# jhorstmann/queryengine

Hardware: AMD Instinct MI355X
Metric: rows/sec filter+project over int64/f64 batch; achieved HBM GB/s in roofline (higher is better)
Workload: dtype int64/f64

## Files before the change

### queryengine_amd/csrc/qe_api.cpp

```cpp
#include <algorithm>
#include <cmath>
#include <cstdio>
#include <cstdlib>
#include <functional>
#include <sstream>

#include "qe_exec.h"
#include "qe_kernels.h"
#include "qe_pernode.h"
#include "qe_scan.h"

using namespace qe;

namespace {

constexpr double kDenseFromSelectivity = 0.12;
constexpr double kLocalUpToSelectivity = 0.03;
constexpr int64_t kSampleFromRows = 8ll << 20;

FusedGeometry geometry_of(const qe_ctx *ctx) {
    FusedGeometry g;
    const int t = ctx->opts.tuning[0], u = ctx->opts.tuning[1];
    if (t == 64 || t == 128 || t == 256 || t == 512 || t == 1024) g.threads = t;
    const int mw = ctx->opts.tuning[3] / 100;
// ... 31 lines not shown
    void partitioned_tile_512_threads();
    void hashed_unroll();
    void dense_lds_tile();
    void ring_lds_budget();
    void register_estimate();
    void compile_without_scratch();
};


}

namespace qe {

std::shared_ptr<Plan> get_plan(qe_ctx *ctx, const qe_batch *batch, const PlanRequest &rq) {
    if (rq.nproj < 0 || (rq.nproj > 0 && !rq.projs)) fail(QE_ERR_INVALID_ARG, "bad projection list");
    CodegenInput in;
    in.filter = rq.filter ? &rq.filter->e : nullptr;
    for (int32_t i = 0; i < rq.nproj; i++) {
        if (!rq.projs[i]) fail(QE_ERR_INVALID_ARG, "null projection");
        in.projections.push_back(&rq.projs[i]->e);
        if (rq.agg_fns) {
            if (rq.agg_fns[i] < QE_AGG_MIN || rq.agg_fns[i] > QE_AGG_AVG) fail(QE_ERR_UNSUPPORTED, "unsupported aggregation function");
            in.agg_fns.push_back(rq.agg_fns[i]);
        }
    }
    for (int32_t i = 0; i < rq.nkeys; i++) {
        if (!rq.keys || !rq.keys[i]) fail(QE_ERR_INVALID_ARG, "null group key");
        in.group_keys.push_back(&rq.keys[i]->e);
    }
    in.cmp_semantics = ctx->opts.cmp_semantics;
    if (rq.conj_order) in.conj_order = *rq.conj_order;
    in.hp_parts = rq.hp_parts;
    static const int lines_maxp = std::getenv("QE_HP_LINES_MAXP") ? std::atoi(std::getenv("QE_HP_LINES_MAXP")) : 512;
    in.hp_lines = !debug_bit(ctx, kDbgHpRecords) && rq.hp_parts <= lines_maxp ? 1 : 0;
    in.hp_shift = rq.hp_shift;
    in.geo = geometry_of(ctx);
    const bool wide = rq.geo_cand == 1;
    if (wide) {
        in.geo.unroll = 16;
        in.geo.subs_per_chunk = 4;
        in.geo.ring_entries = 512;
    } else if (rq.geo_cand == 2) {
        in.geo.unroll = 8;
        in.geo.subs_per_chunk = 8;
        in.geo.ring_entries = 512;
        in.geo.threads = 128;
    }
    in.nontemporal = ctx->opts.tuning[2] % 10 == 2 ? 0 : 1;
    in.vec_stores = ctx->opts.tuning[2] % 10 == 5 ? 1 : 0;
    in.nt_stores = ctx->opts.tuning[2] % 10 == 3 ? 0 : ctx->opts.tuning[2] % 10 == 4 ? 2 : 1;
    in.debug_mask = ctx->opts.tuning[5] & kDbgAblationMask;
    in.staged = !debug_bit(ctx, kDbgNoLateMaterialisation);
    in.prefetch = debug_bit(ctx, kDbgNoPrefetch) ? 0 : debug_bit(ctx, kDbgAlwaysPrefetch) ? 2 : 1;
    in.dense = rq.dense && rq.filter != nullptr && !rq.agg_fns;
    if (in.dense) {
        in.geo.subs_per_chunk = 1;
        in.geo.stagger = 0;
        if (ctx->opts.tuning[0] == 0) in.geo.threads = 256;
        if (ctx->opts.tuning[1] == 0) in.geo.unroll = 8;
    }
    in.filter_load_stages = debug_bit(ctx, kDbgOneFilterLoadStage) ? 1 : 0;
    std::ostringstream key;
    key << "m" << (rq.agg_fns ? 1 : 0) << (in.dense ? "D" : "") << "c" << in.cmp_semantics << "t" << in.geo.threads << "u" << in.geo.unroll << "s"
        << in.geo.subs_per_chunk << "n" << in.nontemporal << in.nt_stores << in.vec_stores << "L" << (in.staged ? 1 : 0) << "P" << in.prefetch << "." << in.filter_load_stages << "k" << in.geo.lookback_k << "G" << in.geo.gate_period_log2 << "." << in.geo.gate_width_log2 << "d" << in.debug_mask << "r" << in.geo.resolve_at << "g" << in.geo.stagger << "w" << in.geo.min_waves << "p" << in.geo.prio_mode << "b" << in.geo.nbuf << "R" << in.geo.ring_entries << "|";
    for (const Column &c : batch->cols) {
        in.schema.push_back(BoundColumn{c.type, c.validity != nullptr, c.dict});
        key << c.type << (c.validity ? 'n' : 'v') << (c.dict ? c.dict->id : 0) << ",";
    }
    auto add_prog = [&](const Expr *e) {
        key << "|";
        if (e) key.write((const char *)e->program.data(), (std::streamsize)e->program.size());
    };
    add_prog(in.filter);
    for (const Expr *e : in.projections) add_prog(e);
    for (const Expr *e : in.group_keys) {
        key << "|k";
        add_prog(e);
    }
    if (rq.agg_fns)
        for (int a : in.agg_fns) key << "|a" << a;
    if (in.hp_parts) key << "|H" << in.hp_parts << "." << in.hp_shift << "." << in.hp_lines;
    if (!in.conj_order.empty()) {
        key << "|O";
        for (int o : in.conj_order) key << o << ".";
    }
    const std::string k = key.str();
    auto it = ctx->plans.find(k);
    if (it != ctx->plans.end() && (it->second->kernel.fn || !rq.load)) return it->second;
    auto plan = std::make_shared<Plan>();
    PlanGeometry pg{ctx, in, plan.get(), wide, rq.agg_fns};
    pg.analyze();
    pg.narrow_plan_wide_candidate();
    pg.lds_table_1024_threads();
    pg.hash_partitioned_tile();
    pg.partitioned_tile_512_threads();
    pg.hashed_unroll();
    pg.dense_lds_tile();
    pg.ring_lds_budget();
    if (ctx->opts.tuning[3] / 100 == 0) {
        pg.register_estimate();
        pg.compile_without_scratch();
    } else {
        plan->cg = generate_fused_source(in);
    }
    plan->geo = in.geo;
    plan->explicit_geometry = ctx->opts.tuning[0] != 0 || ctx->opts.tuning[1] != 0 || ctx->opts.tuning[3] != 0 || ctx->opts.tuning[4] != 0 ||
                              ctx->opts.tuning[7] != 0;
    plan->aggregate = rq.agg_fns != nullptr;
    plan->kernel = ctx->jit->get(plan->cg.source, "qe_fused", rq.load);
    ctx->plans[k] = plan;
    return plan;
}

}

namespace {

// ... 857 lines not shown
```

### queryengine_amd/csrc/qe_codegen.cpp

```cpp
#include "qe_expr_rules.h"

#include <algorithm>
#include <cinttypes>
#include <cmath>
#include <cstdio>
#include <sstream>

namespace qe {

namespace {

const char *kPrelude1 = R"QE(
// ---- generated by libqe_hip: fused filter+project kernel for gfx950 ----
typedef unsigned long long u64;
typedef long long i64;
typedef unsigned int u32;
typedef double  qe_f64x2 __attribute__((ext_vector_type(2)));
typedef i64     qe_i64x2 __attribute__((ext_vector_type(2)));
typedef int     qe_i32x2 __attribute__((ext_vector_type(2)));
typedef u64     u64x2 __attribute__((ext_vector_type(2)));
// Bitmap words (validity, BOOLEAN values) are wave-uniform: read through the constant address space they become SCALAR loads
// (s_load_dwordx4 into SGPRs).  As plain global loads hipcc issued one 16-byte VECTOR load per group and bitmap in which all 64
// lanes fetch the same two words into four VGPRs each -- 48 VGPRs per sub-tile for three nullable columns.  The batch is
// read-only while a kernel runs and the scalar cache starts every kernel invalidated.
// ... 581 lines not shown
            if (a.k.empty()) return a;
            if (n.type == QE_STRING) r.dict = unify(a, b);
            r.v = "(" + a.k + " ? " + a.v + " : " + b.v + ")";
            if (!b.k.empty()) r.k = "(" + a.k + " || " + b.k + ")";
            r.from_int = a.from_int && b.from_int;
            return bind(r);
        }
        case QE_FN_ABS: {
            Val a = emit(e, n.ops[0]);
            r.k = a.k;
            if (n.type == QE_DOUBLE) r.v = "__builtin_fabs(" + a.v + ")";
            else if (n.type == QE_INT64) r.v = "(" + a.v + " < 0 ? (i64)(0ull - (u64)" + a.v + ") : " + a.v + ")";
            else r.v = "(" + a.v + " < 0 ? (int)(0u - (u32)" + a.v + ") : " + a.v + ")";
            r.from_int = a.from_int;
            return bind(r);
        }
        case QE_FN_FLOOR: case QE_FN_CEIL: {
            Val a = emit(e, n.ops[0]);
            if (n.type != QE_DOUBLE) return a;
            r.k = a.k;
            r.v = std::string(n.fn == QE_FN_FLOOR ? "floor(" : "ceil(") + a.v + ")";
            r.from_int = a.from_int;
            return bind(r);
        }
        case QE_FN_IN: case QE_FN_LIKE: return emit_member(e, n, id);
        default: fail(QE_ERR_INTERNAL, "bad function");
        }
    }
};

std::string load_vec_type(int t) {
    switch (t) {
    case QE_DOUBLE: return "qe_f64x2";
    case QE_INT64: return "qe_i64x2";
    default: return "qe_i32x2";
    }
}

void literal_to_dictionary(Val &v) {
    if (!v.is_str_lit) return;
    v.dict = literal_dictionary(v.lit);
    v.v = "0";
    v.is_str_lit = false;
}

enum class FusedForm { FilterProject, Dense, Aggregate, GroupByTable, GroupByPartitioned, GroupByHashed };

struct FusedAnalysis {
    CodegenOutput out;
    FusedForm form = FusedForm::FilterProject;
    bool aggregate = false, groupby = false, has_filter = false;
    bool staged = false;
    bool prefetch = false;
    std::string row_body;
    std::vector<std::string> conj_body;
    std::vector<int> col_stage;
    std::vector<int> vbit;
    std::vector<char> vonly;
    bool any_nullable_in = false;
    bool keys_nullable = false;
    bool member_bits = false, member_hash = false;
    std::string hp_grp_fn;
    HpEntryLayout hp_layout;
    bool row_grp() const { return groupby && !out.hashed; }
    bool row_keys() const { return groupby && (out.hashed || out.hp); }
};

FusedAnalysis analyze_fused(const CodegenInput &in);

struct Emitter {
    const CodegenInput &in;
    const FusedAnalysis &a;
    const CodegenOutput &out;
    const int NC, NO;
    std::ostringstream s;

    Emitter(const CodegenInput &i, const FusedAnalysis &an)
        : in(i), a(an), out(an.out), NC((int)an.out.used_cols.size()), NO((int)an.out.outs.size()) {}
    const BoundColumn &col(int j) const { return in.schema[(size_t)out.used_cols[(size_t)j]]; }

    void header();
    void groupby_macros();
    void access_macros();
    void row_functions();
    std::string valid_arg(int j) const;
    void loads(int stage, bool guarded);
    std::string col_args() const;
    void row_call(bool only_alive);
    void sub_head(const char *intro, const std::string &params, bool filter_project, bool scatter_pass);

    void filter_project();
    void dense();
    void filter_project_head();
    void ring_defs();
    void prefetch_loader();
    void compaction_tail();
    void passthrough_tail();
    void conj_probe();
    void ring_kernel();
    void two_pass_and_local();
    void aggregate();
    void groupby_table();
    void groupby_partitioned();
    void groupby_hashed();
    void hashed_prelude();
    void scatter_save_tail();
    void hashed_build_tail();
    void hashed_accumulate_tail();
    void partitioned_prelude();
    void group_rows_begin();
    void table_accumulate();
    void table_kernel();
    void gb_init_function(const char *comment);
    void merge_entry(const std::string &e);
    void partition_passes();
    void hp_aggregate_pass();
    void range_aggregate_pass();
};

FusedAnalysis analyze_fused(const CodegenInput &in) {
    Gen g(in);
    FusedAnalysis a;
    CodegenOutput &out = a.out;
    if (in.filter) g.mark_used(*in.filter);
    for (const Expr *p : in.projections) g.mark_used(*p);
    for (const Expr *k : in.group_keys) g.mark_used(*k);
    if ((int)g.used_cols.size() > kMaxCols) fail(QE_ERR_UNSUPPORTED, "too many input columns");
    if ((int)in.projections.size() > kMaxOuts) fail(QE_ERR_UNSUPPORTED, "too many projections");
    const bool aggregate = a.aggregate = !in.agg_fns.empty();

    int out_nconj = 0;
    std::vector<std::vector<int>> conj_cols;
    std::vector<int> conj;
    std::vector<std::string> &conj_body = a.conj_body;
    std::vector<int> &col_stage = a.col_stage;
    const bool staged = a.staged = in.filter != nullptr && in.staged && !in.dense;
    std::string keep_expr = "true";
    if (in.filter) {
        if (in.filter->nodes[in.filter->root].type != QE_BOOLEAN)
// ... 145 lines not shown
        out.table_words = 1 + 2 * (int)in.projections.size();
        out.hash_words = 3 + (int)in.group_keys.size() + 2 * (int)in.projections.size();
        {
            int shared = -1;
            for (size_t i = 0; i < out.outs.size(); i++) {
                if (out.outs[i].nullable) { out.cnt_src.push_back((int)i); continue; }
                if (shared < 0) shared = (int)i;
                out.cnt_src.push_back(shared);
            }
        }
        out.table_in_lds = !out.hashed && !out.hp && (size_t)out.ngroups * out.table_words * 8 <= (size_t)(in.geo.threads >= 1024 ? 144 : 48) * 1024;
        out.table_copies = 1;
        if (!out.hashed && !out.table_in_lds && in.projections.size() <= 8) {
            int shift = 0;
            static const size_t table_kb = std::getenv("QE_GB_TABLE_KB") ? (size_t)std::atoi(std::getenv("QE_GB_TABLE_KB")) : 80;
            while (shift < 12 && ((size_t)2 << shift) * out.table_words * 8 <= table_kb * 1024) shift++;
            if (out.hp) shift = out.hp_shift;
            const long long np = (out.ngroups + (1ll << shift) - 1) >> shift;
            if (np <= 1024) {
                for (size_t i = 0; i < in.projections.size(); i++) {
                    int slot = -1;
                    for (size_t j = 0; j < i; j++)
                        if (in.projections[j]->program == in.projections[i]->program) { slot = out.val_slot[j]; break; }
                    if (slot < 0) slot = out.nvals++;
                    out.val_slot.push_back(slot);
                }
                if (out.hp) {
                    out.hp_key_slot = out.nvals;
                    out.nvals += out.hp_key_words;
                    out.hp_line_recs = in.hp_lines ? 128 / (8 * out.nvals + 5) : 0;
                    if (out.hp_line_recs < 2) {
                        out.hp_line_recs = 0;
                        while (((1 + out.nvals) & out.nvals) != 0) out.nvals++;
                    }
                    if (((size_t)1 << out.hp_shift) * (size_t)(out.hp_key_words + 1 + hp_layout.words) * 8 > 156 * 1024)
                        fail(QE_ERR_UNSUPPORTED, "hash-partitioned GROUP BY: entry too wide for an LDS table");
                }
                out.partitioned = true;
                out.part_shift = shift;
                out.part_groups = 1 << shift;
                out.nparts = (int)np;
            }
        }
    }
    const int NC = (int)g.used_cols.size();
    a.vbit.assign((size_t)NC, -1);
    {
        int nn = 0;
        for (int j = 0; j < NC; j++)
            if (in.schema[g.used_cols[j]].nullable) a.vbit[j] = 2 * nn++;
        if (nn > 16) fail(QE_ERR_UNSUPPORTED, "more than 16 nullable input columns in one plan");
        a.any_nullable_in = nn > 0;
    }
    if (!groupby && !aggregate && staged && in.prefetch) {
        bool first = false;
        std::vector<char> has((size_t)conj.size() + 1, 0);
        for (int j = 0; j < NC; j++) { has[(size_t)col_stage[j]] = 1; first = first || col_stage[j] == 0; }
        int nstages = 0;
        for (char h : has) nstages += h ? 1 : 0;
        a.prefetch = first && (in.prefetch >= 2 ? nstages >= 2 : nstages >= 4);
    }
    out.used_cols = g.used_cols;
    out.aux_tables = g.aux;
    if (g.used_cols.size() + g.aux.size() > (size_t)kMaxCols)
        fail(QE_ERR_UNSUPPORTED, "too many input columns + string lookup tables for one fused kernel (use QE_EXEC_PER_NODE)");
    a.has_filter = out.has_filter = in.filter != nullptr;
    out.nconj = out_nconj;
    out.conj_cols = conj_cols;
    for (int j = 0; j < NC; j++) {
        a.vonly.push_back(g.value_used[(size_t)g.used_cols[j]] ? 0 : 1);
        out.col_width.push_back(a.vonly[(size_t)j] ? 0 : value_bytes(in.schema[g.used_cols[j]].type));
    }
    a.row_body = g.body.str();
    a.member_bits = g.uses_member_bits;
    a.member_hash = g.uses_member_hash;
    if (!aggregate) {
        out.dense = in.dense && a.has_filter;
        out.two_pass = a.has_filter && !out.dense;
        out.has_probe = staged && conj.size() >= 2;
        out.fl_ring = std::max(in.geo.ring_entries, output_row_bytes(out.outs) <= 18 ? 512 : 256);
        a.form = out.dense ? FusedForm::Dense : FusedForm::FilterProject;
    } else if (!groupby) {
        a.form = FusedForm::Aggregate;
    } else {
        a.form = out.hashed ? FusedForm::GroupByHashed : out.partitioned ? FusedForm::GroupByPartitioned : FusedForm::GroupByTable;
    }
    return a;
}

void Emitter::header() {
    const FusedGeometry &geo = in.geo;
    const int U = geo.unroll;
    s << "#define QE_LB_K " << geo.lookback_k << "\n#define QE_DEBUG_MASK " << in.debug_mask << "\n#define QE_RESOLVE_AT "
      << geo.resolve_at << "u\n#define QE_MIN_WAVES " << geo.min_waves << "\n#define QE_PRIO_MODE " << geo.prio_mode
      << "\n#define QE_PRIO_MOD " << (geo.prio_mode == 3 ? 2 : 3) << "u\n";
    s << kPrelude1;
    if (a.member_bits) s << kMemberBitsHelper;
    if (a.member_hash) s << kMemberHashHelper;
    s << "#define QE_THREADS " << geo.threads << "\n#define QE_WAVES " << geo.threads / 64 << "\n#define QE_U " << U
      << "\n#define QE_SUB_ROWS " << geo.sub_rows() << "\n#define QE_CHUNK_ROWS " << geo.chunk_rows() << "\n#define QE_SLOT_ROWS "
      << geo.slot_rows() << "\n#define QE_SUBS_PER_CHUNK " << geo.subs_per_chunk << "u\n#define QE_GATE_PERIOD "
      << (geo.gate_period_log2 > 0 ? (1u << geo.gate_period_log2) : 0u) << "u\n#define QE_GATE_WIDTH "
      << (geo.gate_period_log2 > 0 ? (1u << geo.gate_width_log2) : 0u) << "u\n";
}

void Emitter::groupby_macros() {
    s << "#define QE_GB_ADD_U64(p, v) atomicAdd((p), (v))\n#define QE_GB_ADD_F64(p, v) atomicAdd((p), (v))\n"
         "#define QE_GB_MIN_U64(p, v) atomicMin((p), (v))\n#define QE_GB_MIN_I64(p, v) atomicMin((p), (v))\n"
         "#define QE_GB_MAX_I64(p, v) atomicMax((p), (v))\n";
    s << "#define QE_GB_COPIES " << out.table_copies << "\n";
}

void Emitter::hashed_prelude() {
// ... 463 lines not shown
#if QE_GB_LINES
                    {
                        const u32 line = slot / QE_GB_PADU, idx = slot - line * QE_GB_PADU;
                        u64 *ln = L.stage + (size_t)line * 16;
                        if (QE_GB_NV % 2 == 0) {
#pragma unroll
                            for (int v = 0; v < QE_GB_NV; v += 2) {
                                u64x2 rv;
                                rv.x = sv.val[v][u][r];
                                rv.y = sv.val[v + 1 < QE_GB_NV ? v + 1 : v][u][r];
                                *(u64x2 *)(ln + idx * QE_GB_NV + v) = rv;
                            }
                        } else {
#pragma unroll
                            for (int v = 0; v < QE_GB_NV; ++v) ln[idx * QE_GB_NV + v] = sv.val[v][u][r];
                        }
                        ((u32 *)(ln + QE_GB_META))[idx] = (u32)(tile0 + (i64)(wave * QE_SUB_ROWS + u * 128 + 2 * lane + r));
                        if (QE_GB_FLAGS) ((unsigned char *)(ln + QE_GB_META) + 4u * QE_GB_PADU)[idx] = (unsigned char)(w & 255u);
                        if (idx == 0u) L.lineglob[line] = pos / QE_GB_PADU;   // (a run fills its lines from slot 0 on)
                        continue;
                    }
#endif
                    const u64 h = ((u64)pos << 32) | ((u64)(u32)(wave * QE_SUB_ROWS + u * 128 + 2 * lane + r) << (8 + QE_GB_SHIFT)) | ((u64)((w >> 9) & (QE_GB_GP - 1u)) << 8) | (u64)(w & 255u);
                    if (QE_GB_RECW % 2 == 0) {
                        u64x2 rv;
                        rv.x = h;
                        rv.y = sv.val[0][u][r];
                        *(u64x2 *)(L.stage + (size_t)slot * QE_GB_RECW) = rv;
#pragma unroll
                        for (int w = 2; w < QE_GB_RECW; w += 2) {   // record word w (>= 1) is value w - 1
                            u64x2 r2;
                            r2.x = sv.val[w - 1][u][r];
                            r2.y = sv.val[w][u][r];
                            *(u64x2 *)(L.stage + (size_t)slot * QE_GB_RECW + w) = r2;
                        }
                    } else {
                        L.stage[(size_t)slot * QE_GB_RECW] = h;
#pragma unroll
                        for (int v = 0; v < QE_GB_NV; ++v) L.stage[(size_t)slot * QE_GB_RECW + 1 + v] = sv.val[v][u][r];
                    }
                }
            }
        }
    }
}
)QE";
}

void Emitter::access_macros() {
    s << (in.nontemporal ? "#define QE_LD(p) __builtin_nontemporal_load(p)\n" : "#define QE_LD(p) (*(p))\n");
    s << (in.nt_stores ? "#define QE_ST(p, v) __builtin_nontemporal_store((v), (p))\n" : "#define QE_ST(p, v) (*(p) = (v))\n");
    s << (in.nt_stores == 2 ? "#define QE_SPILL_ST(p, v) __builtin_nontemporal_store((v), (p))\n" : "#define QE_SPILL_ST(p, v) (*(p) = (v))\n");
    s << "#define QE_VEC_ST " << (in.vec_stores ? 1 : 0) << "\n";
}

void Emitter::row_functions() {
    for (size_t ci = 0; ci < a.conj_body.size(); ci++) {
        s << "\n__device__ __forceinline__ void qe_conj" << ci << "(const QeParams &p, ";
        for (int j = 0; j < NC; j++) {
            const BoundColumn &bc = col(j);
            s << "const " << ctype(bc.type) << " c" << j << ", ";
            if (bc.nullable) s << "const bool kc" << j << ", ";
        }
        s << "bool &alive) {\n    (void)p;\n";
        for (int j = 0; j < NC; j++) {
            s << "    (void)c" << j << ";";
            if (col(j).nullable) s << " (void)kc" << j << ";";
        }
        s << "\n" << a.conj_body[ci] << "}\n";
    }
    s << "\n__device__ __forceinline__ void qe_row(const QeParams &p";
    bool first = false;
    for (int j = 0; j < NC; j++) {
        const BoundColumn &bc = col(j);
        s << (first ? "" : ", ") << "const " << ctype(bc.type) << " c" << j;
        first = false;
        if (bc.nullable) s << ", const bool kc" << j;
    }
    s << (first ? "" : ", ") << "bool &keep";
    for (int i = 0; i < NO; i++) {
        s << ", " << ctype(out.outs[i].type) << " &o" << i;
        if (out.outs[i].nullable) s << ", bool &ok" << i;
    }
    if (a.row_grp()) s << ", int &grp";
    if (a.row_keys()) {
        for (size_t i = 0; i < in.group_keys.size(); i++) s << ", u64 &kw" << i;
        s << ", u32 &knull";
    }
    s << ") {\n    (void)p;\n" << a.row_body << "}\n";
}

void Emitter::ring_defs() {
    const FusedGeometry &geo = in.geo;
    s << "\n#define QE_NBUF " << geo.nbuf << "u\n#define QE_RING " << geo.ring_entries << "   // LDS entries per wave, buffer and output column (power of two)\n";
    s << "#define QE_FL_RING " << out.fl_ring << "\n";
    s << "struct QeRing {\n";
    for (int i = 0; i < NO; i++) {
        const OutSpec &os = out.outs[i];
        s << "    " << (os.type == QE_BOOLEAN ? "unsigned char" : ctype(os.type)) << " *r" << i << ";\n";
        if (os.nullable) s << "    unsigned char *rv" << i << ";\n";
    }
    if (NO == 0) s << "    int unused;\n";
    s << "};\n";
}

std::string Emitter::valid_arg(int j) const { return "((qe_vb[u] >> (" + std::to_string(a.vbit[j]) + " + r)) & 1u) != 0u"; }

void Emitter::loads(int stage, bool guarded) {
    s << "#pragma unroll\n    for (int u = 0; u < QE_U; ++u) {\n";
    s << "        const i64 r0 = sub0 + u * 128 + 2 * lane;\n";
    s << "        const i64 g0 = (sub0 + u * 128) >> 6;   // wave-uniform bitmap word index (even)\n";
    s << "        const u32 sh = (u32)(2 * lane) & 63u;\n";
    s << "        const i64 nwords = (p.nrows + 63) >> 6;\n        (void)nwords; (void)g0; (void)sh; (void)r0;\n";
    if (guarded) s << "        if (keep[u][0] || keep[u][1]) {\n";
    for (int j = 0; j < NC; j++) {
        if (stage >= 0 && a.col_stage[j] != stage) continue;
        const BoundColumn &bc = col(j);
        auto bitmap_load = [&](const std::string &ptr, const std::string &dst, int vb = -1) {
            s << "        {\n            const qe_cu64p bm = (qe_cu64p)(u64)(" << ptr << ");\n";
            s << "            u64 w0, w1;\n";
            s << "            if (FULL) { w0 = bm[g0]; w1 = bm[g0 + 1]; }\n";
            s << "            else { w0 = g0 < nwords ? bm[g0] : 0ull; w1 = g0 + 1 < nwords ? bm[g0 + 1] : 0ull; }\n";
            s << "            const u64 w = lane < 32 ? w0 : w1;\n";
            if (vb >= 0) {
                s << "            qe_vb[u] |= ((u32)(w >> sh) & 3u) << " << vb << ";\n        }\n";
            } else {
                s << "            " << dst << "[u][0] = (w >> sh) & 1ull;\n";
                s << "            " << dst << "[u][1] = (w >> (sh + 1u)) & 1ull;\n        }\n";
            }
        };
        if (a.vonly[(size_t)j]) {
            const std::string ct = bc.type == QE_BOOLEAN ? "bool" : ctype(bc.type);
            s << "        c" << j << "[u][0] = (" << ct << ")0; c" << j << "[u][1] = (" << ct << ")0;\n";
        } else if (bc.type == QE_BOOLEAN) {
            bitmap_load("(const u64 *)p.col[" + std::to_string(j) + "]", "c" + std::to_string(j));
        } else {
            const std::string ct = ctype(bc.type), vt = load_vec_type(bc.type);
            s << "        {\n            const " << ct << " *src = (const " << ct << " *)p.col[" << j << "] + r0;\n";
            s << "            if (FULL) { const " << vt << " v = QE_LD((const " << vt << " *)src); c" << j
              << "[u][0] = v.x; c" << j << "[u][1] = v.y; }\n";
            s << "            else { c" << j << "[u][0] = r0 < p.nrows ? src[0] : (" << ct << ")0; c" << j
              << "[u][1] = r0 + 1 < p.nrows ? src[1] : (" << ct << ")0; }\n        }\n";
        }
        if (bc.nullable) bitmap_load("p.colvalid[" + std::to_string(j) + "]", "", a.vbit[j]);
    }
    if (guarded) s << "        }\n";
    s << "    }\n";
}

void Emitter::prefetch_loader() {
    bool s0_nulls = false;
    s << "\nstruct QeS0 {\n";
    for (int j = 0; j < NC; j++) {
        if (a.col_stage[j] != 0) continue;
        const BoundColumn &bc = col(j);
        s << "    " << (bc.type == QE_BOOLEAN ? "bool" : ctype(bc.type)) << " c" << j << "[QE_U][2];\n";
        s0_nulls = s0_nulls || bc.nullable;
    }
    if (s0_nulls) s << "    u32 vb[QE_U];\n";
    s << "};\n// issue the stage-0 loads of the (full) sub-tile at sub0\n"
         "__device__ __forceinline__ void qe_s0_load(const QeParams &p, const i64 sub0, const int lane, QeS0 &s0) {\n"
         "    constexpr bool FULL = true;\n";
    for (int j = 0; j < NC; j++)
        if (a.col_stage[j] == 0) s << "    auto &c" << j << " = s0.c" << j << ";\n";
    if (s0_nulls) s << "    auto &qe_vb = s0.vb;\n#pragma unroll\n    for (int u = 0; u < QE_U; ++u) qe_vb[u] = 0u;\n";
    loads(0, false);
    s << "}\n";
}

std::string Emitter::col_args() const {
    std::string args;
    for (int j = 0; j < NC; j++) {
        args += (args.empty() ? "" : ", ") + std::string("c") + std::to_string(j) + "[u][r]";
        if (col(j).nullable) args += ", " + valid_arg(j);
    }
    return args;
}

void Emitter::row_call(bool only_alive) {
    s << "#pragma unroll\n    for (int u = 0; u < QE_U; ++u) {\n#pragma unroll\n        for (int r = 0; r < 2; ++r) {\n";
    const std::string ca = col_args();
    if (only_alive) s << "            if (keep[u][r]) {\n                bool unused_keep;\n                qe_row(p, " << ca << (ca.empty() ? "" : ", ") << "unused_keep";
    else s << "            qe_row(p, " << ca << (ca.empty() ? "" : ", ") << "keep[u][r]";
    for (int i = 0; i < NO; i++) {
        s << ", o" << i << "[u][r]";
        if (out.outs[i].nullable) s << ", ok" << i << "[u][r]";
    }
    if (a.row_grp()) s << ", grp[u][r]";
    if (a.row_keys()) {
        for (size_t i = 0; i < in.group_keys.size(); i++) s << ", kw" << i << "[u][r]";
        s << ", knull[u][r]";
    }
    s << ");\n";
    if (only_alive) s << "                (void)unused_keep;\n            }\n";
    else s << "            if (!FULL) keep[u][r] = keep[u][r] && (sub0 + u * 128 + 2 * lane + r < p.nrows);\n";
    s << "        }\n    }\n";
}

const char *kPlainSubIntro = "\ntemplate <bool FULL, typename Hook>\n__device__ __forceinline__ void qe_sub(const QeParams &p, const i64 sub0, const int lane, Hook &&after_loads";

void Emitter::sub_head(const char *intro, const std::string &params, bool filter_project, bool scatter_pass) {
    s << intro << params << ") {\n";
    s << "    bool keep[QE_U][2];\n";
    if (a.row_grp()) s << "    int grp[QE_U][2];\n";
    if (a.row_keys()) {
        for (size_t i = 0; i < in.group_keys.size(); i++) s << "    u64 kw" << i << "[QE_U][2];\n";
        s << "    u32 knull[QE_U][2];\n";
    }
    for (int i = 0; i < NO; i++) {
        s << "    " << ctype(out.outs[i].type) << " o" << i << "[QE_U][2];\n";
        if (out.outs[i].nullable) s << "    bool ok" << i << "[QE_U][2];\n";
    }
    for (int j = 0; j < NC; j++) {
        const BoundColumn &bc = col(j);
        if (bc.type == QE_BOOLEAN) s << "    bool c" << j << "[QE_U][2];\n";
        else s << "    " << ctype(bc.type) << " c" << j << "[QE_U][2];\n";
    }
    if (a.any_nullable_in) s << "    u32 qe_vb[QE_U] = {};\n";
    if (!a.staged) {
        if (filter_project) s << "    (void)pf; (void)next_sub0;\n";
        loads(-1, false);
        s << "    after_loads();   // stores and polls of earlier work are issued here, under the loads just started\n";
        row_call(false);
    } else {
        const int K = (int)a.conj_body.size();
        for (int st = 0; st <= K; st++) {
            bool any = false;
            for (int j = 0; j < NC; j++) any = any || a.col_stage[j] == st;
            if (st == 0) {
                if (a.prefetch) {
                    s << "    if (PF) {   // stage 0 is in `pf` already; start the next sub-tile's stage 0 right away\n";
                    bool s0_nulls = false;
                    for (int j = 0; j < NC; j++) {
                        if (a.col_stage[j] != 0) continue;
                        s << "#pragma unroll\n        for (int u = 0; u < QE_U; ++u) { c" << j << "[u][0] = pf.c" << j << "[u][0]; c" << j << "[u][1] = pf.c" << j << "[u][1]; }\n";
                        s0_nulls = s0_nulls || col(j).nullable;
                    }
                    if (s0_nulls) s << "#pragma unroll\n        for (int u = 0; u < QE_U; ++u) qe_vb[u] = pf.vb[u];\n";
                    s << "        if (next_sub0 >= 0) qe_s0_load(p, next_sub0, lane, pf);\n    } else {\n";
                }
                loads(0, false);
                if (a.prefetch) s << "    }\n";
                if (!a.prefetch && filter_project) s << "    (void)pf; (void)next_sub0;\n";
                if (scatter_pass) {
                    s << "    if (MODE == 2) {\n";
                    for (int later = 1; later <= K; later++) {
                        bool has = false;
                        for (int j = 0; j < NC; j++) has = has || a.col_stage[j] == later;
                        if (has) loads(later, false);
                    }
                    s << "    }\n";
                }
                s << "    after_loads();   // stores and polls of earlier work are issued here, under the loads just started\n";
            } else if (any) {
                if (scatter_pass) s << "    if (MODE != 2) {\n";
                loads(st, true);
                if (scatter_pass) s << "    }\n";
            }
            if (st == K) break;
            s << "#pragma unroll\n    for (int u = 0; u < QE_U; ++u) {\n#pragma unroll\n        for (int r = 0; r < 2; ++r) {\n";
            const std::string ca = col_args();
            if (st == 0) {
                s << "            bool alive;\n            qe_conj0(p, " << ca << (ca.empty() ? "" : ", ") << "alive);\n";
                s << "            if (!FULL) alive = alive && (sub0 + u * 128 + 2 * lane + r < p.nrows);\n";
                s << "            keep[u][r] = alive;\n";
            } else {
                s << "            if (keep[u][r]) {\n                bool alive;\n                qe_conj" << st << "(p, " << ca << (ca.empty() ? "" : ", ")
                  << "alive);\n                keep[u][r] = alive;\n            }\n";
            }
            s << "        }\n    }\n";
        }
        row_call(true);
    }
}

void Emitter::scatter_save_tail() {
    s << "    if (MODE == 2) {   // keep the evaluated sub-tile: it is sorted and written under the next sub-tile's loads\n"
         "        sv.sub0 = sub0;\n#pragma unroll\n        for (int u = 0; u < QE_U; ++u) {\n#pragma unroll\n            for (int r = 0; r < 2; ++r) {\n"
         "                u32 w = ((u32)grp[u][r] << 9) | 256u;\n";
    for (int i = 0; i < NO; i++) {
        std::string cond = out.outs[i].nullable ? "ok" + std::to_string(i) + "[u][r]" : "true";
        s << "                if (" << cond << ") w |= " << (1u << i) << "u;\n";
    }
    s << "                sv.w[u][r] = keep[u][r] ? w : 0u;\n";
    {
        std::vector<std::string> slot_val((size_t)out.nvals);
        for (int i = NO - 1; i >= 0; i--) slot_val[out.val_slot[i]] = "__builtin_bit_cast(u64, (double)o" + std::to_string(i) + "[u][r])";
        if (out.hp) {
            for (int kk = 0; kk < (int)in.group_keys.size(); kk++) slot_val[(size_t)(out.hp_key_slot + kk)] = "kw" + std::to_string(kk) + "[u][r]";
            if (out.hp_key_words > (int)in.group_keys.size()) slot_val[(size_t)(out.hp_key_slot + out.hp_key_words - 1)] = "(u64)knull[u][r]";
        }
        for (int v = 0; v < out.nvals; v++) s << "                sv.val[" << v << "][u][r] = " << (slot_val[v].empty() ? std::string("0ull") : slot_val[v]) << ";\n";
    }
    s << "            }\n        }\n        return;\n    }\n";
}

void Emitter::hashed_build_tail() {
    s << "    if (MODE == 1) {\n        u32 id[QE_U][2];\n        u64 hh[QE_U][2], st[QE_U][2], ekn[QE_U][2], eid[QE_U][2], ek[QE_U][2][QE_HT_NK];\n        bool miss[QE_U][2];\n"
         "#pragma unroll\n        for (int u = 0; u < QE_U; ++u) {\n#pragma unroll\n            for (int r = 0; r < 2; ++r) {\n"
         "                miss[u][r] = keep[u][r]; id[u][r] = 0u; hh[u][r] = 0ull; st[u][r] = 0ull; ekn[u][r] = 0ull; eid[u][r] = 0ull;\n"
         "                if (keep[u][r]) {\n                    u64 key[QE_HT_NK];\n";
    for (size_t i = 0; i < in.group_keys.size(); i++) s << "                    key[" << i << "] = kw" << i << "[u][r];\n";
    s << "                    hh[u][r] = qe_ht_hash(key, (u64)knull[u][r]);\n"
         "                }\n            }\n        }\n"
         "        // up to 8 slots of the probe sequence, every pending row's loads in flight together per step\n"
         "        bool pend[QE_U][2], found[QE_U][2];\n        u32 slot[QE_U][2];\n"
         "#pragma unroll\n        for (int u = 0; u < QE_U; ++u) {\n#pragma unroll\n            for (int r = 0; r < 2; ++r) {\n"
         "                pend[u][r] = miss[u][r]; found[u][r] = false; slot[u][r] = (u32)hh[u][r] & ((u32)p.capacity - 1u) & ~3u;   // probe sequences start on a 4-entry group: one 128-byte line\n            }\n        }\n"
         "        if (QE_HT_NK == 1) {\n"
         "#pragma unroll\n            for (int u = 0; u < QE_U; ++u) {\n#pragma unroll\n                for (int r = 0; r < 2; ++r) slot[u][r] = (u32)hh[u][r] & ((u32)p.capacity - 1u) & ~7u;\n            }\n"
         "#pragma unroll\n            for (int d = 0; d < 8; ++d) {\n"
         "                bool anyp = false;\n"
         "#pragma unroll\n                for (int u = 0; u < QE_U; ++u) anyp = anyp || pend[u][0] || pend[u][1];\n"
         "                if (__ballot(anyp) == 0ull || (QE_DEBUG_MASK & 2)) break;\n"
         "#pragma unroll\n                for (int u = 0; u < QE_U; ++u) {\n#pragma unroll\n                    for (int r = 0; r < 2; ++r)\n"
         "                        if (pend[u][r]) { const u64x2 t = *(const u64x2 *)(gtab + (size_t)slot[u][r] * 2); ek[u][r][0] = t.x; st[u][r] = t.y; }\n                }\n"
         "                asm volatile(\"\" ::: \"memory\");\n"
         "#pragma unroll\n                for (int u = 0; u < QE_U; ++u) {\n#pragma unroll\n                    for (int r = 0; r < 2; ++r) {\n"
         "                        if (!pend[u][r]) continue;\n"
         "                        const u64 m = st[u][r];\n"
         "                        if ((m & 3ull) != 2ull) { pend[u][r] = false; continue; }   // empty, unfinished or a stale copy: the coherent path decides\n"
         "                        if (ek[u][r][0] == kw0[u][r] && ((m >> 8) & 0xffull) == (u64)knull[u][r]) { found[u][r] = true; pend[u][r] = false; eid[u][r] = m >> 32; }\n"
         "                        else slot[u][r] = (slot[u][r] + 1u) & ((u32)p.capacity - 1u);\n"
         "                    }\n                }\n            }\n"
         "        } else {\n"
// ... 1520 lines not shown
```

### queryengine_amd/csrc/qe_internal.h

```cpp
#pragma once

#include <hip/hip_runtime_api.h>

#include <cstdint>
#include <cstring>
#include <map>
#include <memory>
#include <string>
#include <unordered_map>
#include <vector>

#include "../../include/qe_hip.h"

namespace qe {

struct Error {
    int32_t code;
    std::string msg;
};
[[noreturn]] void fail(int32_t code, const std::string &msg);
void hip_check(hipError_t e, const char *what, const char *file, int line);
#define QE_HIP(x) ::qe::hip_check((x), #x, __FILE__, __LINE__)

enum NodeKind { N_COLUMN = 0, N_NUM = 1, N_BOOL = 2, N_STR = 3, N_FN = 4, N_CAST = 5, N_LIST = 6 };
// ... 160 lines not shown
    bool nullable;
    std::shared_ptr<DictData> dict;
};

struct OutSpec {
    int type;
    bool nullable;
    std::shared_ptr<DictData> dict;
};

inline int value_bytes(int type) { return type == QE_BOOLEAN ? 0 : (type == QE_DOUBLE || type == QE_INT64) ? 8 : 4; }
inline size_t output_row_bytes(const std::vector<OutSpec> &outs) {
    size_t n = 0;
    for (const OutSpec &o : outs) n += (o.type == QE_BOOLEAN ? 1 : value_bytes(o.type)) + (o.nullable ? 1 : 0);
    return n;
}

struct FusedGeometry {
    int threads = 256;
    int rows_per_lane = 2;
    int unroll = 8;
    int subs_per_chunk = 16;
    int nbuf = 2;
    int ring_entries = 256;
    int lookback_k = 1;
    int gate_period_log2 = 0;
    int gate_width_log2 = 0;
    int stagger = 0;
    int min_waves = 4;
    int prio_mode = 1;
    int resolve_at = 1;
    int sub_rows() const { return 64 * rows_per_lane * unroll; }
    int chunk_rows() const { return sub_rows() * subs_per_chunk; }
    int slot_rows() const { return chunk_rows() + 832; }
};

struct CodegenInput {
    const Expr *filter = nullptr;
    std::vector<const Expr *> projections;
    std::vector<int> agg_fns;
    std::vector<const Expr *> group_keys;
    std::vector<BoundColumn> schema;
    int cmp_semantics = QE_CMP_TOTAL_ORDER;
    FusedGeometry geo;
    int nontemporal = 1;
    int vec_stores = 0;
    int nt_stores = 1;
    int hp_shift = 0;
    int hp_lines = 1;
    int hp_parts = 0;
    std::vector<int> conj_order;
    int filter_load_stages = 0;
    int prefetch = 1;
    bool staged = true;
    bool dense = false;
    int debug_mask = 0;
};

struct CodegenOutput {
    std::string source;
    std::vector<OutSpec> outs;
    std::vector<int> used_cols;
    bool has_filter = false;
    bool two_pass = false;
    bool dense = false;
    bool has_probe = false;
    int nconj = 0;
    std::vector<std::vector<int>> conj_cols;
    std::vector<int> col_width;
    int fl_ring = 0;
    std::vector<std::vector<int32_t>> aux_tables;
    std::vector<OutSpec> keys;
    std::vector<int> key_domain;
    long long ngroups = 0;
    int table_words = 0;
    bool table_in_lds = false;
    bool hashed = false;
    int hash_words = 0;
    int table_copies = 1;
    std::vector<int> cnt_src;
    bool partitioned = false;
    int part_shift = 0;
    int part_groups = 0;
    int nparts = 0;
    std::vector<int> val_slot;
    int nvals = 0;
    bool hp = false;
    int hp_key_words = 0, hp_key_slot = 0, hp_shift = 11;
    int hp_line_recs = 0;
};

CodegenOutput generate_fused_source(const CodegenInput &in);
CodegenOutput analyze_fused_plan(const CodegenInput &in);

struct Kernel {
    hipModule_t module = nullptr;
    hipFunction_t fn = nullptr;
    int scratch = -1;
};

class Jit {
public:
    explicit Jit(std::string cache_dir) : cache_dir_(std::move(cache_dir)) {}
    ~Jit();
    Kernel get(const std::string &source, const char *entry, bool load = true);
    void reject(const std::string &source, int scratch);
// ... 109 lines not shown
        bool nullable = false;
        void *data = nullptr;
        uint64_t *validity = nullptr;
        std::shared_ptr<qe::DictData> dict;
        qe_dict dict_handle;
    };
    std::vector<Col> cols;
    hipEvent_t done = nullptr;
    bool waited = false;
};

namespace qe {

class __attribute__((visibility("hidden"))) PoolScratch {
public:
    explicit PoolScratch(qe_ctx *ctx) : ctx_(ctx) {}
    PoolScratch(const PoolScratch &) = delete;
    PoolScratch &operator=(const PoolScratch &) = delete;
    ~PoolScratch() { for (void *p : bufs_) ctx_->pool.release(p); }
    void *alloc(size_t bytes) {
        bufs_.push_back(nullptr);
        return bufs_.back() = ctx_->pool.alloc(bytes);
    }

private:
    qe_ctx *ctx_;
    std::vector<void *> bufs_;
};

enum DebugBit : int {
    kDbgAblationMask = 255,
    kDbgWaitStats = 16,
    kDbgTrace = 32,
    kDbgScatterClocks = 64,
    kDbgGroupByGlobalAtomics = 256,
    kDbgForceTwoPass = 512,
    kDbgNeverTwoPass = 1024,
    kDbgNoLateMaterialisation = 2048,
    kDbgOneFilterLoadStage = 4096,
    kDbgNoGeometryChoice = 8192,
    kDbgForceDense = 16384,
    kDbgNeverDense = 32768,
    kDbgNoSelectivitySample = 65536,
    kDbgHashedGlobalAtomics = 131072,
    kDbgForceLocal = 262144,
    kDbgNeverLocal = 524288,
    kDbgWrittenConjunctOrder = 1048576,
    kDbgNoPrefetch = 2097152,
    kDbgAlwaysPrefetch = 4194304,
    kDbgForceHashPartitioned = 8388608,
    kDbgNeverHashPartitioned = 16777216,
    kDbgHpRecords = 33554432,
    kDbgGroupsOnDevice = 67108864,
};
inline bool debug_bit(const qe_ctx *ctx, DebugBit b) { return (ctx->opts.tuning[5] & b) != 0; }

inline int32_t last_stats(const qe_ctx *ctx, Stats4 qe_ctx::*which, int64_t out[4]) {
    if (!ctx || !out) return QE_ERR_INVALID_ARG;
    for (int i = 0; i < 4; i++) out[i] = (ctx->*which).w[i];
    return QE_OK;
}

}

std::vector<int64_t> qe_int_count_slices(qe_ctx *ctx, const qe_batch *batch, const qe_expr *filter, const qe_expr *const *projs, int32_t nproj,
                                         int64_t *slice_rows_io, int32_t nslices);
qe_result *qe_int_run_fused_slice(qe_ctx *ctx, const qe_batch *batch, int64_t row_begin, int64_t nrows, const qe_expr *filter,
                                  const qe_expr *const *projs, int32_t nproj);
```

Before: 324.6 billion.

## Use buffer loads with out-of-range dead lanes for late-stage column loads

For staged filter plans with late-materialised value columns, the generated kernel now builds a per-sub-tile buffer descriptor and loads columns with raw buffer loads. Dead lanes get an offset past the descriptor range, so the hardware returns zero for them without a per-lane branch. A wave-level ballot also skips a whole stage's loads when no row is still alive. This is meant to cut divergent-branch overhead and wasted HBM traffic for filtered-out rows. By default it applies only when there are at least four stages, and it adds descriptor setup and readfirstlane work.

```diff
diff --git a/queryengine_amd/csrc/qe_api.cpp b/queryengine_amd/csrc/qe_api.cpp
--- a/queryengine_amd/csrc/qe_api.cpp
+++ b/queryengine_amd/csrc/qe_api.cpp
@@ -107,6 +107,7 @@
     in.debug_mask = ctx->opts.tuning[5] & kDbgAblationMask;
     in.staged = !debug_bit(ctx, kDbgNoLateMaterialisation);
     in.prefetch = debug_bit(ctx, kDbgNoPrefetch) ? 0 : debug_bit(ctx, kDbgAlwaysPrefetch) ? 2 : 1;
+    in.late_loads = debug_bit(ctx, kDbgBranchGuardedLoads) ? 0 : debug_bit(ctx, kDbgAlwaysBufferLoads) ? 2 : 1;
     in.dense = rq.dense && rq.filter != nullptr && !rq.agg_fns;
     if (in.dense) {
         in.geo.subs_per_chunk = 1;
@@ -117,7 +118,7 @@
     in.filter_load_stages = debug_bit(ctx, kDbgOneFilterLoadStage) ? 1 : 0;
     std::ostringstream key;
     key << "m" << (rq.agg_fns ? 1 : 0) << (in.dense ? "D" : "") << "c" << in.cmp_semantics << "t" << in.geo.threads << "u" << in.geo.unroll << "s"
-        << in.geo.subs_per_chunk << "n" << in.nontemporal << in.nt_stores << in.vec_stores << "L" << (in.staged ? 1 : 0) << "P" << in.prefetch << "." << in.filter_load_stages << "k" << in.geo.lookback_k << "G" << in.geo.gate_period_log2 << "." << in.geo.gate_width_log2 << "d" << in.debug_mask << "r" << in.geo.resolve_at << "g" << in.geo.stagger << "w" << in.geo.min_waves << "p" << in.geo.prio_mode << "b" << in.geo.nbuf << "R" << in.geo.ring_entries << "|";
+        << in.geo.subs_per_chunk << "n" << in.nontemporal << in.nt_stores << in.vec_stores << "L" << (in.staged ? 1 : 0) << "P" << in.prefetch << "." << in.filter_load_stages << "B" << in.late_loads << "k" << in.geo.lookback_k << "G" << in.geo.gate_period_log2 << "." << in.geo.gate_width_log2 << "d" << in.debug_mask << "r" << in.geo.resolve_at << "g" << in.geo.stagger << "w" << in.geo.min_waves << "p" << in.geo.prio_mode << "b" << in.geo.nbuf << "R" << in.geo.ring_entries << "|";
     for (const Column &c : batch->cols) {
         in.schema.push_back(BoundColumn{c.type, c.validity != nullptr, c.dict});
         key << c.type << (c.validity ? 'n' : 'v') << (c.dict ? c.dict->id : 0) << ",";
diff --git a/queryengine_amd/csrc/qe_codegen.cpp b/queryengine_amd/csrc/qe_codegen.cpp
--- a/queryengine_amd/csrc/qe_codegen.cpp
+++ b/queryengine_amd/csrc/qe_codegen.cpp
@@ -657,6 +657,7 @@
     bool aggregate = false, groupby = false, has_filter = false;
     bool staged = false;
     bool prefetch = false;
+    bool buffer_loads = false;
     std::string row_body;
     std::vector<std::string> conj_body;
     std::vector<int> col_stage;
@@ -690,6 +691,9 @@
     void row_functions();
     std::string valid_arg(int j) const;
     void loads(int stage, bool guarded);
+    void load_loop(int stage, int mode);
+    bool buffer_loaded(int j) const;
+    bool buffer_loads() const;
     std::string col_args() const;
     void row_call(bool only_alive);
     void sub_head(const char *intro, const std::string &params, bool filter_project, bool scatter_pass);
@@ -941,13 +945,17 @@
         if (nn > 16) fail(QE_ERR_UNSUPPORTED, "more than 16 nullable input columns in one plan");
         a.any_nullable_in = nn > 0;
     }
-    if (!groupby && !aggregate && staged && in.prefetch) {
+    if (staged) {
         bool first = false;
         std::vector<char> has((size_t)conj.size() + 1, 0);
         for (int j = 0; j < NC; j++) { has[(size_t)col_stage[j]] = 1; first = first || col_stage[j] == 0; }
         int nstages = 0;
         for (char h : has) nstages += h ? 1 : 0;
-        a.prefetch = first && (in.prefetch >= 2 ? nstages >= 2 : nstages >= 4);
+        if (!groupby && !aggregate && in.prefetch) a.prefetch = first && (in.prefetch >= 2 ? nstages >= 2 : nstages >= 4);
+        bool late_values = false;
+        for (int j = 0; j < NC; j++)
+            late_values = late_values || (col_stage[j] > 0 && g.value_used[(size_t)g.used_cols[j]] && in.schema[g.used_cols[j]].type != QE_BOOLEAN);
+        a.buffer_loads = late_values && (in.late_loads >= 2 || (in.late_loads == 1 && nstages >= 4));
     }
     out.used_cols = g.used_cols;
     out.aux_tables = g.aux;
@@ -1517,6 +1525,16 @@
     s << (in.nt_stores ? "#define QE_ST(p, v) __builtin_nontemporal_store((v), (p))\n" : "#define QE_ST(p, v) (*(p) = (v))\n");
     s << (in.nt_stores == 2 ? "#define QE_SPILL_ST(p, v) __builtin_nontemporal_store((v), (p))\n" : "#define QE_SPILL_ST(p, v) (*(p) = (v))\n");
     s << "#define QE_VEC_ST " << (in.vec_stores ? 1 : 0) << "\n";
+    if (buffer_loads()) {
+        const char *aux = in.nontemporal ? "2 /* nt */" : "0";
+        s << "#define QE_BLD16(rs, off) __builtin_amdgcn_raw_buffer_load_b128((rs), (off), 0, " << aux << ")\n"
+             "#define QE_BLD8(rs, off) __builtin_amdgcn_raw_buffer_load_b64((rs), (off), 0, " << aux << ")\n"
+             "// descriptor of `bytes` bytes at `base`; the base goes through readfirstlane so that the descriptor is provably wave-uniform\n"
+             "__device__ __forceinline__ __amdgpu_buffer_rsrc_t qe_sub_rsrc(const void *base, const u32 bytes) {\n"
+             "    const u64 b = (u64)base;\n"
+             "    const u64 ub = ((u64)(u32)__builtin_amdgcn_readfirstlane((int)(b >> 32)) << 32) | (u64)(u32)__builtin_amdgcn_readfirstlane((int)(u32)b);\n"
+             "    return __builtin_amdgcn_make_buffer_rsrc((void *)ub, 0, (int)bytes, 0x00020000);\n}\n";
+    }
 }
 
 void Emitter::row_functions() {
@@ -1572,12 +1590,33 @@
 std::string Emitter::valid_arg(int j) const { return "((qe_vb[u] >> (" + std::to_string(a.vbit[j]) + " + r)) & 1u) != 0u"; }
 
 void Emitter::loads(int stage, bool guarded) {
+    if (guarded && buffer_loads()) {
+        s << "    if (FULL) {\n";
+        for (int j = 0; j < NC; j++)
+            if (a.col_stage[j] == stage && buffer_loaded(j))
+                s << "        const __amdgpu_buffer_rsrc_t rs" << j << " = qe_sub_rsrc((const " << ctype(col(j).type) << " *)p.col[" << j
+                  << "] + sub0, (u32)(QE_SUB_ROWS * sizeof(" << ctype(col(j).type) << ")));\n";
+        load_loop(stage, 2);
+        s << "    } else {\n";
+        load_loop(stage, 1);
+        s << "    }\n";
+        return;
+    }
+    load_loop(stage, guarded ? 1 : 0);
+}
+
+bool Emitter::buffer_loaded(int j) const { return !a.vonly[(size_t)j] && col(j).type != QE_BOOLEAN; }
+bool Emitter::buffer_loads() const { return a.buffer_loads; }
+
+void Emitter::load_loop(int stage, int mode) {
+    const bool guarded = mode == 1;
     s << "#pragma unroll\n    for (int u = 0; u < QE_U; ++u) {\n";
     s << "        const i64 r0 = sub0 + u * 128 + 2 * lane;\n";
     s << "        const i64 g0 = (sub0 + u * 128) >> 6;   // wave-uniform bitmap word index (even)\n";
     s << "        const u32 sh = (u32)(2 * lane) & 63u;\n";
     s << "        const i64 nwords = (p.nrows + 63) >> 6;\n        (void)nwords; (void)g0; (void)sh; (void)r0;\n";
     if (guarded) s << "        if (keep[u][0] || keep[u][1]) {\n";
+    if (mode == 2) s << "        const u32 row = (keep[u][0] || keep[u][1]) ? (u32)(u * 128 + 2 * lane) : 0x10000000u;   // a dead lane: past the descriptor's range\n";
     for (int j = 0; j < NC; j++) {
         if (stage >= 0 && a.col_stage[j] != stage) continue;
         const BoundColumn &bc = col(j);
@@ -1599,6 +1638,10 @@
             s << "        c" << j << "[u][0] = (" << ct << ")0; c" << j << "[u][1] = (" << ct << ")0;\n";
         } else if (bc.type == QE_BOOLEAN) {
             bitmap_load("(const u64 *)p.col[" + std::to_string(j) + "]", "c" + std::to_string(j));
+        } else if (mode == 2) {
+            const std::string ct = ctype(bc.type), vt = load_vec_type(bc.type);
+            s << "        {\n            const " << vt << " v = __builtin_bit_cast(" << vt << ", " << (value_bytes(bc.type) == 8 ? "QE_BLD16" : "QE_BLD8")
+              << "(rs" << j << ", row * (u32)sizeof(" << ct << ")));\n            c" << j << "[u][0] = v.x; c" << j << "[u][1] = v.y;\n        }\n";
         } else {
             const std::string ct = ctype(bc.type), vt = load_vec_type(bc.type);
             s << "        {\n            const " << ct << " *src = (const " << ct << " *)p.col[" << j << "] + r0;\n";
@@ -1689,6 +1732,7 @@
         row_call(false);
     } else {
         const int K = (int)a.conj_body.size();
+        int open_blocks = 0;
         for (int st = 0; st <= K; st++) {
             bool any = false;
             for (int j = 0; j < NC; j++) any = any || a.col_stage[j] == st;
@@ -1718,9 +1762,15 @@
                 }
                 s << "    after_loads();   // stores and polls of earlier work are issued here, under the loads just started\n";
             } else if (any) {
+                if (buffer_loads()) {
+                    s << "    bool live" << st << " = false;\n#pragma unroll\n    for (int u = 0; u < QE_U; ++u) live" << st << " = live" << st
+                      << " || keep[u][0] || keep[u][1];\n    if (!FULL || __ballot(live" << st << ") != 0ull) {\n";
+                    open_blocks++;
+                }
                 if (scatter_pass) s << "    if (MODE != 2) {\n";
                 loads(st, true);
                 if (scatter_pass) s << "    }\n";
+                for (; open_blocks > 0; open_blocks--) s << "    }\n";
             }
             if (st == K) break;
             s << "#pragma unroll\n    for (int u = 0; u < QE_U; ++u) {\n#pragma unroll\n        for (int r = 0; r < 2; ++r) {\n";
@@ -1736,6 +1786,7 @@
             s << "        }\n    }\n";
         }
         row_call(true);
+        for (int i = 0; i < open_blocks; i++) s << "    }\n";
     }
 }
 
diff --git a/queryengine_amd/csrc/qe_internal.h b/queryengine_amd/csrc/qe_internal.h
--- a/queryengine_amd/csrc/qe_internal.h
+++ b/queryengine_amd/csrc/qe_internal.h
@@ -236,6 +236,7 @@
     std::vector<int> conj_order;
     int filter_load_stages = 0;
     int prefetch = 1;
+    int late_loads = 1;
     bool staged = true;
     bool dense = false;
     int debug_mask = 0;
@@ -451,6 +452,8 @@
     kDbgNeverHashPartitioned = 16777216,
     kDbgHpRecords = 33554432,
     kDbgGroupsOnDevice = 67108864,
+    kDbgBranchGuardedLoads = 134217728,
+    kDbgAlwaysBufferLoads = 268435456,
 };
 inline bool debug_bit(const qe_ctx *ctx, DebugBit b) { return (ctx->opts.tuning[5] & b) != 0; }
 
```

Result: slower. 309.2 billion (-4.8%).
